# lunarlab-gatech/MorphSym-HGNN

Hardware: AMD Instinct MI355X
Metric: graph-windows/sec fwd+bwd, A1-C2 GRF regression (higher is better)
Workload: dtype bf16; 1 GPU; A1-C2 GRF regression (3-D), h=128, L=3, T=150, 8192 windows/GPU, fwd+MSE+bwd, all parameter gradients; global_batch=8192, parallelism=dp1, rccl_ranks=0

## Files before the change

### morphsym_hgnn_amd/csrc/mshgnn.hip

```cpp
#include "mshgnn_slab.hpp"
#include "mshgnn_enc.hpp"
#include "mshgnn_launch.hpp"
extern "C" const char* mshgnn_last_error(void) { return g_err.c_str(); }
extern "C" const char* mshgnn_version(void) { return "mshgnn 0.5 (gfx950)"; }
extern "C" int mshgnn_abi_version(void) { return MSHGNN_ABI_VERSION; }
extern "C" size_t mshgnn_struct_size(int which) {
    switch (which) {
        case 0: return sizeof(mshgnn_desc);
        case 1: return sizeof(mshgnn_info);
        case 2: return sizeof(mshgnn_ws_layout);
        case 3: return sizeof(mshgnn_window_desc);
        case 4: return sizeof(mshgnn_kernel_stat);
        case 5: return sizeof(mshgnn_mlp_desc);
        case 6: return sizeof(mshgnn_mlp_info);
        case 7: return sizeof(mshgnn_mlp_input);
        default: return 0;
    }
}


template <typename T> __device__ __forceinline__ void prep_one(const PrepArgs& a, int idx, bool with_bias) {
    constexpr int EPC = Prec<T>::EPC, NBV = Prec<T>::NBV;
    const int vec_per_pack = H * H / EPC;
    const int npk = a.pack_n < 0 ? a.n_packs : a.pack_n;
// ... 912 lines not shown

#ifndef GW_WPS
#define GW_WPS 3
#endif

template <bool ALIGNED, bool SERIES = false> __global__ __launch_bounds__(256, GW_WPS) void k_gradw_bf16_lean(GradwArgs a) {
    static_assert(!SERIES || ALIGNED, "the series gather replaces the aligned raw loads");
    using T = __bf16;
    __shared__ __attribute__((aligned(16))) __bf16 Ps[GWB_KW * GWB_PITCH];
    __shared__ __attribute__((aligned(16))) __bf16 Qs[GWB_KW * GWB_PITCH];
    __shared__ __attribute__((aligned(16))) u32x4 mlut[256];
    __shared__ __attribute__((aligned(16))) u32x4 qkeep_t[16];
    __shared__ __attribute__((aligned(16))) u32x4 qsign_t[GW_IPL][16];
    __shared__ unsigned long long sbase[GW_IPL][4];
    __shared__ unsigned long long sser[SERIES ? GW_IPL : 1][16][2];
    const int tid = threadIdx.x, lane = tid & 63, wv = __builtin_amdgcn_readfirstlane(tid >> 6);
    mlut[tid] = chunk_mask_bits<__bf16>(u32x4{0xffffffffu, 0xffffffffu, 0xffffffffu, 0xffffffffu}, (unsigned)tid);
    const int wr = wv >> 1, wc = wv & 1;
    const int ln = a.lane_order[blockIdx.x % a.n_pad], part = blockIdx.x / a.n_pad;
    if (ln < 0) return;
    const int* lh = a.lanes + ln * LANE_INTS;
    const int it0 = lh[0], nit = lh[1] - lh[0], bias_flag = lh[3];
    const int* im0 = a.items + it0 * ITEM_INTS;
    const int nchunks = (a.B + GWB_KW - 1) / GWB_KW;
    const int ch0 = (int)((int64_t)part * nchunks / a.n_parts), ch1 = (int)((int64_t)(part + 1) * nchunks / a.n_parts);
    const int nsteps = ch1 - ch0, total = nsteps * nit;
    const int c = tid & 15, r4 = (tid >> 4) * 4;

    const bool p_masked = im0[9] >= 0, q_raw = im0[4] < 0;
    const int ntile = (a.B + 15) >> 4;
    const unsigned voffP = (unsigned)(r4 * H + c * 8) * (unsigned)sizeof(T);
    const unsigned voffM = (unsigned)(((c >> 2) * ntile + (r4 >> 4)) * 64 + (c & 3) * 16 + (r4 & 15));
    const int qt = q_raw ? im0[3] - BUF_IN : 0;
    const unsigned qsb = q_raw ? (unsigned)(a.nodes[qt] * a.pitch[qt]) * (unsigned)sizeof(T) : (unsigned)(H * sizeof(T));
// ... 163 lines not shown
        for (int e = 0; e < 8; ++e) red[(r4 >> 2) * H + c * 8 + e] = bsum[e];
        __syncthreads();
        if (tid < H) {
            float s2 = 0.f;
#pragma unroll
            for (int r = 0; r < 16; ++r) s2 += red[r * H + tid];
            slab[H * H + tid] = s2;
        }
    }
}


#ifndef FIN_LB
#define FIN_LB 4
#endif
__global__ __launch_bounds__(256) void k_finalize(FinArgs a) {
    const int* f = a.fin + blockIdx.x * FIN_INTS;
    const int64_t dst = (int64_t)(unsigned)f[0] | ((int64_t)f[1] << 32);
    const int rows = f[2], cols = f[3], ld = f[4], tg = f[5], kind = f[6];
    const int* more = f[7] ? a.fin0 + f[7] : nullptr;
    const int RPB = (rows + gridDim.y - 1) / gridDim.y;
    const int r0 = blockIdx.y * RPB, r1 = min(rows, r0 + RPB);
    const int n = (r1 - r0) * cols;
    if (a.loss && blockIdx.x == 0 && blockIdx.y == 0 && threadIdx.x < 64) {
        float l = 0.f;
        for (int b = threadIdx.x; b < a.n_dec; b += 64) l += a.dec_slabs[(size_t)b * DEC_SLAB_FLOATS + 8 * H + 8];
#pragma unroll
        for (int m = 32; m >= 1; m >>= 1) l += __shfl_xor(l, m, 64);
        if (threadIdx.x == 0) *a.loss = l * a.inv_n + (a.accumulate ? *a.loss : 0.f);
    }
    if (!a.grad) return;
// ... 260 lines not shown
    if (prep_use_tiled(a.n_packs)) hipLaunchKernelGGL((k_prep_tiled<T, false>), dim3(prep_tiled_grid(a.n_packs, a.n_biases)), dim3(256), 0, st, a);
    else hipLaunchKernelGGL(k_prep<T>, dim3(prep_grid(a, Prec<T>::EPC, biases)), dim3(256), 0, st, a);
}
int launch_prep(const PrepArgs& a, bool split, hipStream_t st) {
    if (split) x3_launch_prep(a, true, st); else launch_prep_t<__bf16>(a, true, st);
    return MSHGNN_OK;
}

int run_finalize(const mshgnn_plan* p, const StepCall& c, const mshgnn_ws_layout& lay, int gw_parts) {
    const HostPlan& hp = p->hp;
    const mshgnn_desc& d = hp.d;
    char* ws = c.ws; float* gparams = c.grad_params; hipStream_t st = c.stream;
    const int B = (int)c.batch, gw_phase = c.gw_phase;
    float* loss = c.loss != LossKind::NONE ? c.loss_out : nullptr;
    FinArgs a{p->d_tables + hp.fin_off, p->d_tables + hp.fin_off, p->d_tables + hp.tgt_off, reinterpret_cast<const float*>(ws + lay.slabs),
              reinterpret_cast<const float*>(ws + lay.dec_slabs), gparams, hp.n_lanes, gw_parts, loss,
              1.0f / (float)(c.total_windows() * d.type_nodes[d.out_type] * (c.loss == LossKind::CE ? 1 : d.out_channels)),
              c.dec_done ? (int)((B + TILE_ROWS - 1) / TILE_ROWS) : NWG_DEC, c.accumulates()};
    int f0 = 0, nf = hp.n_fin;
    if (gw_phase == 0) nf = hp.n_fin_ph0;
    if (gw_phase == 1) { f0 = hp.n_fin_ph0; nf = hp.n_fin - hp.n_fin_ph0; a.loss = nullptr; }
    a.fin += (size_t)f0 * FIN_INTS;
    if (!gparams) {
        if (loss) hipLaunchKernelGGL(k_finalize, dim3(1, 1), dim3(256), 0, st, a);
        HIPCHK(hipGetLastError());
        return MSHGNN_OK;
    }
    ProfScope ps(p, hp.ks_fin, st);
    if (nf > 0) hipLaunchKernelGGL(k_finalize, dim3(nf, 64), dim3(256), 0, st, a);
    HIPCHK(hipGetLastError());
    return MSHGNN_OK;
}

template <typename T> static constexpr LaunchTraits plan_traits{
    (int)sizeof(T), Prec<T>::EPC, Prec<T>::EPC, Prec<T>::BLK, Prec<T>::ENC_MB * Prec<T>::ROWS, Prec<T>::ENC_MB * Prec<T>::BLK, sizeof(T) == 4 ? GW_KW : GWB_KW,
     false,  sizeof(T) == 2,  sizeof(T) == 2,  false,  sizeof(T) == 2,
    "the fused window assembly needs 16-byte aligned window rows (pitch a multiple of 8)",
    "wide source rows: the plan-dtype rows need 16-byte alignment and a pitch that is a multiple of 8"};

template <typename T>
static int forward_impl(const mshgnn_plan* p, StepCall& c) {
    const HostPlan& hp = p->hp;
    const mshgnn_desc& d = hp.d;
    const LaunchTraits& tr = plan_traits<T>;
// ... 77 lines not shown
    for (int l = hp.L - 1; l >= 0 && !fused_done; --l) {
        LayerArgs a{};
        a.x_in = ws + lay.dx[l + 1]; a.x_out = ws + lay.dx[l]; a.maskbits = reinterpret_cast<unsigned*>(ws + lay.mask[l]);
        a.hb = ws + lay.hb[l]; a.t1 = ws + lay.t1[l]; a.dh = ws + lay.dh[l]; a.du = ws + lay.du[l]; a.x_act = ws + lay.x[0];
        a.wpack = ws + lay.wpack; a.bias = reinterpret_cast<const float*>(ws + lay.bias);
        a.prog = p->d_tables + hp.bwd_prog_off[l]; a.B = B; a.NN = hp.NN; a.n_mlp = std::max(1, hp.n_mlp);
        a.dbg = p->dbg;
        ProfScope ps(p, hp.ks_layer_bwd0 + (hp.L - 1 - l), st);
        hipLaunchKernelGGL(k_layer_bwd<T>, dim3(tiles), dim3(LAYER_THREADS), hp.n_blk * Prec<T>::BLK, st, a);
    }
    const int gw_parts = gw_parts_for(hp.n_parts, hp.n_lanes, hp.gw_ipl, B, tr.gw_windows, p->n_cu);
    if (c.grad_params) {
        GradwArgs a{};
        fill_gradw_args(p, c, lay, tr, gw_parts, a);
        ProfScope ps(p, hp.ks_gradw, st);
        const dim3 grid(std::max(a.n_pad, 0) * gw_parts);
        if (a.n_pad <= 0) {}
        else if constexpr (sizeof(T) == 4) hipLaunchKernelGGL(k_gradw_f32, grid, dim3(256), 0, st, a);
        else if (c.gradw_from_series && c.series) hipLaunchKernelGGL((k_gradw_bf16_lean<true, true>), grid, dim3(256), 0, st, a);
        else if (a.aligned) hipLaunchKernelGGL(k_gradw_bf16_lean<true>, grid, dim3(256), 0, st, a);
        else hipLaunchKernelGGL(k_gradw_bf16_lean<false>, grid, dim3(256), 0, st, a);
    }
    return run_finalize(p, c, lay, gw_parts);
}

static int run_forward(const mshgnn_plan* p, StepCall& c) {
    if (c.wide && c.series) return set_err(MSHGNN_EINVAL, "a call takes its encoder rows from wide sources or from a series, not from both");
    if (p->gen) return gen_forward(p, c);
    if (p->hp.d.dtype == MSHGNN_BF16X3) return x3_forward(p, c);
    if (p->hp.d.dtype == MSHGNN_F32) return forward_impl<float>(p, c);
    return forward_impl<__bf16>(p, c);
}
// ... 452 lines not shown
```

### morphsym_hgnn_amd/csrc/mshgnn_device.hpp

```cpp
#pragma once
#include <type_traits>
#include <hip/hip_runtime.h>

#include <cmath>
#include <cstdio>
#include <cstdlib>
#include <cstring>
#include <string>
#include <vector>

#include "mshgnn_plan.hpp"

using namespace mshgnn;

typedef float f32x4 __attribute__((ext_vector_type(4)));
typedef float f32x2 __attribute__((ext_vector_type(2)));
typedef float f32x16 __attribute__((ext_vector_type(16)));
typedef __bf16 bf16x8 __attribute__((ext_vector_type(8)));
typedef unsigned int u32x4 __attribute__((ext_vector_type(4)));
typedef double f64x2 __attribute__((ext_vector_type(2)));
typedef unsigned int u32x2 __attribute__((ext_vector_type(2)));

#ifndef ENC_NT
#define ENC_NT 0
// ... 1229 lines not shown
template <typename T, int THREADS, bool SPLIT = false, bool TOLDS = false>
__device__ __forceinline__ void decoder_tail(const StackArgs& a, char* smem, int tid, int lane, int wv, int w0, int B) {
    if (a.dout <= 4) decoder_tail_impl<T, THREADS, 4, SPLIT, TOLDS>(a, smem, tid, lane, wv, w0, B);
    else decoder_tail_impl<T, THREADS, 8, SPLIT, TOLDS>(a, smem, tid, lane, wv, w0, B);
}
constexpr int DEC_NPP_STATIC = 4;

struct DecArgs {
    const void* xl; void* dxl; const float* params; const float* out_mask; float* out; const float* gout; float* slabs;
    int64_t off_w, off_b; int B, NN, node0, n_out, dout, slab0;
    const float* y; float* loss; float inv_n;
    const int32_t* labels;
};


struct GradwArgs {
    const char* ws; size_t buf_off[BUF_COUNT];
    const void* x[MSHGNN_MAX_TYPES]; int64_t pitch[MSHGNN_MAX_TYPES]; int nodes[MSHGNN_MAX_TYPES]; int vb[MSHGNN_MAX_TYPES];
    const int* items; const int* lanes; const int* lane_order; const uint8_t* signs; float* slabs; int B, n_lanes, n_parts, n_pad;
    int aligned;
    int dbg; long long* stamps;
    SeriesSrc ser;
};

constexpr int GWB_KW = 64;
constexpr int GWB_PITCH = 128;
__device__ __forceinline__ int gwb_elem(int row, int col) { return row * GWB_PITCH + ((((col >> 3) ^ ((row & 3) << 2)) << 3) | (col & 7)); }
typedef short s16x4 __attribute__((ext_vector_type(4)));

__device__ __forceinline__ bf16x8 tr_frag(const __bf16* tile, int w_base, int col_base, int lane) {
    const int g = lane >> 4, q = (lane >> 2) & 3, pp = lane & 3;
    const __bf16* p0 = tile + gwb_elem(w_base + 8 * (g >> 1) + q, col_base + 16 * (g & 1) + 4 * pp);
    const s16x4 lo = __builtin_amdgcn_ds_read_tr16_b64_v4i16((__attribute__((address_space(3))) s16x4*)(p0));
    const s16x4 hi = __builtin_amdgcn_ds_read_tr16_b64_v4i16((__attribute__((address_space(3))) s16x4*)(p0 + 4 * GWB_PITCH));
    typedef short s16x8 __attribute__((ext_vector_type(8)));
    const s16x8 v = {lo[0], lo[1], lo[2], lo[3], hi[0], hi[1], hi[2], hi[3]};
    return __builtin_bit_cast(bf16x8, v);
}


struct FinArgs { const int* fin; const int* fin0; const int* targets; const float* slabs; const float* dec_slabs; float* grad; int n_lanes, n_parts; float* loss; float inv_n;
                 int n_dec; int accumulate; };

struct mshgnn_gen_state;
struct ProfRec { int slot; hipEvent_t a, b; };
struct mshgnn_plan {
    HostPlan hp;
    bool prof = false;
    std::vector<ProfRec> recs;
    std::vector<hipEvent_t> free_events;
    int* d_tables = nullptr; uint8_t* d_signs = nullptr; float* d_out_mask = nullptr;
    PackDesc* d_packs = nullptr; BiasDesc* d_biases = nullptr;
    int* d_ig_nodes = nullptr;
    bool attr_set = false;
    bool use_fused = false;
    bool use_slab = false;
    bool slab_force = false; int n_cu = 256;
// ... 116 lines not shown
```

### morphsym_hgnn_amd/csrc/mshgnn_hostplan.cpp

```cpp
#include "mshgnn_plan.hpp"
#include "mshgnn_gen_plan.hpp"
#include "mshgnn_pick.hpp"

using namespace mshgnn;

namespace {
thread_local std::string g_hp_err;

std::string check_tables(const HostPlan& p) {
    char buf[256];
    auto bad = [&](const char* what, int l, int v, int lim) { snprintf(buf, sizeof buf, "%s: layer %d value %d limit %d", what, l, v, lim); return std::string(buf); };
    const int n_packs = (int)p.packs.size() * (p.split ? 2 : 1), n_bias = (int)p.biases.size();
    auto check_prog = [&](int off, int hs, int cb, int nblk, const char* what, int l) -> std::string {
        const int32_t* pr = p.tables.data() + off;
        if (off < 0 || off + FPROG_LEN > (int)p.tables.size()) return bad("program offset", l, off, (int)p.tables.size());
        auto at = [&](int i) { return (pr[128 + (i >> 2)] >> ((i & 3) << 3)) & 0xff; };
        const int nseg = at(0);
        if (nseg > 64) return bad("segments", l, nseg, 64);
        int pb = 1;
        for (int s = 0; s < nseg; ++s) {
            if (pr[s] < 0 || pr[s] >= n_packs) return bad(what, l, pr[s], n_packs);
            for (int u = 0; u < hs; ++u) pb += (pr[64 + s] >> (cb * u)) & ((1 << cb) - 1);
            if (hs * cb < 32 && (pr[64 + s] >> (hs * cb)) != 0) return bad("count bits beyond the slots", l, pr[64 + s], 0);
        }
// ... 105 lines not shown
    for (int i = 0; i < n_items; ++i) {
        const int32_t* it = T + p.item_off + i * GITEM_INTS;
        if (it[I_PBUF] < 0 || it[I_PBUF] >= GBUF_COUNT) return bad("item P buffer", i, it[I_PBUF], GBUF_COUNT);
        if (it[I_SRC0] < 0 || it[I_NSRC] < 1 || it[I_SRC0] + it[I_NSRC] > n_srcs) return bad("item source range", i, it[I_SRC0] + it[I_NSRC], n_srcs);
        { const std::string e = check_srcs(it[I_SRC0], it[I_NSRC], it[I_KIND], "item", i); if (!e.empty()) return e; }
    }
    return "";
}
}

extern "C" {

const char* mshgnn_hostplan_last_error() { return g_hp_err.c_str(); }

enum { HPM_OK = 0, HPM_L, HPM_NN, HPM_NMLP, HPM_FUSED, HPM_SLAB, HPM_SL_HB, HPM_SL_BLK, HPM_FS_BLK, HPM_NTABLES, HPM_NPACKS, HPM_NBIASES, HPM_SL_ALIAS, HPM_NITEMS, HPM_NLANES, HPM_NFIN,
       HPM_SL_FWD = 16, HPM_SL_BWD = 32, HPM_FS_FWD = 48, HPM_FS_BWD = 64, HPM_LIVE = 80 , HPM_NEED = 112, HPM_X3_ALIAS = 144, HPM_SPLIT = 145, HPM_COUNT = 160 };

int mshgnn_hostplan_compile(const mshgnn_desc* desc, int32_t* tables, int cap, int32_t* meta, int check) {
    HostPlan hp;
    if (!compile_plan(desc, hp)) { g_hp_err = hp.err; return -1; }
    if (check) { const std::string e = check_tables(hp); if (!e.empty()) { g_hp_err = "table check: " + e; return -2; } }
    if (meta) {
        std::memset(meta, 0, sizeof(int32_t) * HPM_COUNT);
        meta[HPM_OK] = 1; meta[HPM_L] = hp.L; meta[HPM_NN] = hp.NN; meta[HPM_NMLP] = hp.n_mlp; meta[HPM_FUSED] = hp.fused; meta[HPM_SLAB] = hp.slab; meta[HPM_SL_HB] = hp.sl_hb;
        meta[HPM_SL_BLK] = hp.sl_blk; meta[HPM_FS_BLK] = hp.fs_blk; meta[HPM_NTABLES] = (int)hp.tables.size(); meta[HPM_NPACKS] = (int)hp.packs.size(); meta[HPM_NBIASES] = (int)hp.biases.size();
        meta[HPM_X3_ALIAS] = hp.x3_alias; meta[HPM_SPLIT] = hp.split;
        meta[HPM_SL_ALIAS] = hp.sl_alias; meta[HPM_NITEMS] = hp.n_items; meta[HPM_NLANES] = hp.n_lanes; meta[HPM_NFIN] = hp.n_fin;
        for (int l = 0; l < hp.L; ++l) {
            meta[HPM_SL_FWD + l] = hp.sl_fwd_off[l]; meta[HPM_SL_BWD + l] = hp.sl_bwd_off[l]; meta[HPM_FS_FWD + l] = hp.fs_fwd_off[l]; meta[HPM_FS_BWD + l] = hp.fs_bwd_off[l];
            uint64_t lv = 0, nd = 0;
            for (int n = 0; n < hp.NN; ++n) { lv |= (uint64_t)(hp.live_n[l][n] ? 1 : 0) << n; nd |= (uint64_t)(hp.need_n[l][n] ? 1 : 0) << n; }
            meta[HPM_LIVE + 2 * l] = (int32_t)(uint32_t)lv; meta[HPM_LIVE + 2 * l + 1] = (int32_t)(uint32_t)(lv >> 32);
            meta[HPM_NEED + 2 * l] = (int32_t)(uint32_t)nd; meta[HPM_NEED + 2 * l + 1] = (int32_t)(uint32_t)(nd >> 32);
        }
    }
    if (tables) std::memcpy(tables, hp.tables.data(), sizeof(int32_t) * std::min<size_t>(cap > 0 ? cap : 0, hp.tables.size()));
    return (int)hp.tables.size();
}

int mshgnn_hostplan_compile_gen(const mshgnn_desc* desc, int32_t* meta, int check) {
    gen::GenPlan gp;
    if (!gen::compile_gen_plan(desc, gp)) { g_hp_err = gp.err; return -1; }
// ... 66 lines not shown
```

### morphsym_hgnn_amd/csrc/mshgnn_launch.hpp

```cpp
#pragma once
#include "mshgnn_device.hpp"
#include "mshgnn_pick.hpp"

struct LaunchTraits {
    int in_bytes;
    int in_epc;
    int pack_epc;
    int blk;
    int enc_windows;
    int enc_lds;
    int gw_windows;
    bool split;
    bool embed_prep;
    bool src_routes;
    bool wide_needs_rows;
    bool gradw_series;
    const char* series_rows_err;
    const char* wide_rows_err;
};

inline int plan_packs(const HostPlan& hp, const LaunchTraits& tr) { return tr.split ? hp.n_img : (int)hp.packs.size(); }

using PrepLaunch = void (*)(const PrepArgs&, bool biases, hipStream_t);
inline unsigned prep_grid(const PrepArgs& a, int pack_epc, bool biases) {
// ... 120 lines not shown
inline int forward_op(const StepCall& c) { return c.dec_done ? pick::OP_FWD_LOSS : c.training ? pick::OP_FWD_TRAIN : pick::OP_FWD_EVAL; }
inline void apply_stack_pick(const HostPlan& hp, const pick::StackPick& pk, const mshgnn_ws_layout& lay, StackArgs& a) {
    const int* fwd = pk.slab_prog ? hp.sl_fwd_off : hp.fs_fwd_off;
    const int* bwd = pk.slab_prog ? hp.sl_bwd_off : hp.fs_bwd_off;
    for (int l = 0; l < hp.L; ++l) { a.prog_off[l] = pk.what == pick::BWD ? bwd[l] : fwd[l]; if (pk.what == pick::STEP) a.prog_off_b[l] = bwd[l]; }
    if (pk.what != pick::FWD) a.mask0_off = lay.dd[0];
    a.red_off = pk.red_off; a.stash_nt = pk.stash_nt; a.stagger = pk.stagger;
}
inline int launch_stack(StackKernelFn kernel, const pick::StackPick& pk, hipStream_t st, const StackArgs& a) {
    if (!kernel) return set_err(MSHGNN_EHIP, std::string("no kernel in the launch table for ") + pick::kernel_name(pk.family, pk.k));
    hipLaunchKernelGGL(kernel, dim3(pk.tiles), dim3(pk.threads), pk.lds, st, a);
    HIPCHK(hipGetLastError());
    return MSHGNN_OK;
}

inline void fill_gradw_args(const mshgnn_plan* p, const StepCall& c, const mshgnn_ws_layout& lay, const LaunchTraits& tr, int gw_parts, GradwArgs& a) {
    const HostPlan& hp = p->hp;
    const mshgnn_desc& d = hp.d;
    a.ws = c.ws;
    for (int l = 0; l <= hp.L; ++l) { a.buf_off[BUF_X + l] = lay.x[l]; a.buf_off[BUF_DX + l] = lay.dx[l]; }
    for (int l = 0; l < hp.L; ++l) a.buf_off[BUF_MASK + l] = lay.mask[l];
    for (int l = 0; l < hp.L; ++l) { a.buf_off[BUF_DH + l] = lay.dh[l]; a.buf_off[BUF_HB + l] = lay.hb[l]; a.buf_off[BUF_T1 + l] = lay.t1[l]; a.buf_off[BUF_DU + l] = lay.du[l]; }
    for (int t = 0; t < hp.NT; ++t) {
        a.x[t] = c.x ? c.x[t] : nullptr; a.pitch[t] = c.x_pitch ? c.x_pitch[t] : d.type_width[t]; a.nodes[t] = d.type_nodes[t];
        a.vb[t] = vec_bytes(a.x[t], a.pitch[t], tr.in_bytes);
        if (t == 0) a.aligned = 1;
        if (a.vb[t] != 16 || a.pitch[t] % tr.in_epc) a.aligned = 0;
    }
    if (tr.gradw_series && c.gradw_from_series && c.series) a.ser = *c.series;
    a.items = p->d_tables + hp.item_off; a.lanes = p->d_tables + hp.lane_off; a.lane_order = p->d_tables + hp.lane_order_off; a.n_pad = hp.n_lanes_pad;
    if (c.gw_phase >= 0) { a.lane_order = p->d_tables + hp.order_ph_off[c.gw_phase]; a.n_pad = hp.npad_ph[c.gw_phase]; }
    a.signs = p->d_signs; a.slabs = reinterpret_cast<float*>(c.ws + lay.slabs); a.B = (int)c.batch; a.n_lanes = hp.n_lanes; a.n_parts = gw_parts;
}
```

### morphsym_hgnn_amd/csrc/mshgnn_plan.hpp

```cpp
#pragma once
#include <algorithm>
#include <array>
#include <cmath>
#include <cstdint>
#include <cstdio>
#include <cstring>
#include <string>
#include <vector>

#include "../../include/mshgnn.h"

#ifdef MSHGNN_TUNING
#define TUNE_ENV(name) std::getenv(name)
#else
#define TUNE_ENV(name) (static_cast<const char*>(nullptr))
#endif

namespace mshgnn {

constexpr int H = 128;
constexpr int GMAX = 12;
constexpr int TILE_ROWS = 16;
constexpr int MAX_L = 16;
#ifndef LDS_LIMIT_KB
// ... 36 lines not shown
       FH_SLOTA = 8 + 4 * FS_MAXN,
       FH_SLOTB = FH_SLOTA + 16,
       FH_SIZE = FH_SLOTB + 16,
       FH_NEXT = FH_SLOTA };
static_assert(FH_NEXT + 8 + 20 <= FH_SIZE && MSHGNN_MAX_TYPES <= 4, "header: next-layer array");
constexpr int SL_HA = 12, SL_HB = 6, SL_HB_MAX = 8, SL_THREADS = 256;
constexpr int SL_CBA = 2, SL_CBB = 3;
enum { FF_RESIDUAL = 1, FF_ENC_MASK = 2, FF_SCR_ALIAS = 4, FF_A_EMPTY = 8, FF_B_EMPTY = 16 };

enum { BUF_X = 0, BUF_DX = 17, BUF_DH = 34, BUF_HB = 50, BUF_T1 = 66, BUF_DU = 82, BUF_IN = 98, BUF_MASK = 102, BUF_COUNT = 118 };
constexpr int ITEM_INTS = 10;
constexpr int TGT_INTS = 8;
constexpr int LANE_INTS = 4;
constexpr int FIN_INTS = 8;
enum { FIN_MATRIX = 0, FIN_BIAS = 1, FIN_ZERO = 2, FIN_DEC_W = 3, FIN_DEC_B = 4 };

struct PackDesc {
    int orient;
    int n_src;
    int64_t src[8];
    int ld;
    int col0;
    int ncols;
};
struct BiasDesc { int n_src; int64_t src[8]; };

struct HostPlan {
    mshgnn_desc d{};
    void* jit_prog = nullptr;
    std::vector<int32_t> rel_src, rel_dst, rel_mean, rel_edge_off, edges;
// ... 30 lines not shown
    std::vector<int32_t> tables;
    int fwd_prog_off[MAX_L]{}, bwd_prog_off[MAX_L]{};
    bool fused = false;
    int fs_fwd_off[MAX_L]{}, fs_bwd_off[MAX_L]{};
    bool slab = false;
    int sl_fwd_off[MAX_L]{}, sl_bwd_off[MAX_L]{}, sl_ta = -1, sl_hb = SL_HB, sl_blk = 0;
    bool sl_alias = false;
    int fs_blk = 0;
    bool x3_alias = false;
    int ks_stack_fwd = -1, ks_stack_bwd = -1;
    int item_off = 0, n_items = 0, tgt_off = 0, n_targets = 0, lane_off = 0, n_lanes = 0, n_parts = 1, n_wg_gradw = 0;
    int lane_order_off = 0, n_lanes_pad = 0, gw_ipl = 1;
    int order_ph_off[2]{}, npad_ph[2]{}, n_fin_ph0 = 0;
    int64_t grad_split = -1;
    int fin_off = 0, n_fin = 0;
    int enc_tile_mb = 4;
    int n_slabs = 0;
    std::vector<float> out_mask_f;
    std::vector<mshgnn_kernel_stat> kstats;
    int ks_prep = 0, ks_enc = 0, ks_layer_fwd0 = 0, ks_dec_fwd = 0, ks_dec_bwd = 0, ks_layer_bwd0 = 0, ks_gradw = 0, ks_fin = 0, ks_stack_step = 0;
    mshgnn_info info{};
    std::string err;
};

inline bool fail(HostPlan& p, const std::string& m) { p.err = m; return false; }

inline int add_pack(HostPlan& p, int orient, const std::vector<int64_t>& src, int ld, int col0, int ncols) {
    PackDesc q{}; q.orient = orient; q.n_src = (int)src.size(); q.ld = ld; q.col0 = col0; q.ncols = ncols;
    for (size_t i = 0; i < src.size(); ++i) q.src[i] = src[i];
    p.packs.push_back(q); return (int)p.packs.size() - 1;
// ... 843 lines not shown
        std::vector<int32_t> extra;
        for (auto& f : fins) {
            if (!is_ph1(f)) ++p.n_fin_ph0;
            if (is_ph1(f) && f.target >= 0 && !tgt_is_enc[f.target]) p.grad_split = -1;
            for (int64_t m : f.more) if ((p.grad_split >= 0 && m < p.grad_split) != is_ph1(f)) p.grad_split = -1;
            T.push_back((int32_t)(f.dst & 0xffffffff)); T.push_back((int32_t)(f.dst >> 32)); T.push_back(f.rows); T.push_back(f.cols);
            T.push_back(f.ld); T.push_back(f.target); T.push_back(f.kind);
            T.push_back(f.more.empty() ? 0 : (int32_t)(fins.size() * FIN_INTS + extra.size()));
            if (!f.more.empty()) {
                extra.push_back((int32_t)f.more.size());
                for (int64_t m : f.more) { extra.push_back((int32_t)(m & 0xffffffff)); extra.push_back((int32_t)(m >> 32)); }
            }
        }
        T.insert(T.end(), extra.begin(), extra.end());
        if (p.grad_split < 0) p.n_fin_ph0 = p.n_fin;
    }

    p.info.rows_per_tile = p.rows; p.info.total_nodes = p.NN; p.info.lds_bytes = (int64_t)p.n_blk * p.blk_bytes;
    p.info.flops_fwd = alg_fwd; p.info.flops_bwd = alg_bwd; p.info.flops_exec_fwd = exec_fwd; p.info.flops_exec_bwd = exec_bwd;
    double bytes = 0, bytes_all = 0;
    for (int t = 0; t < NT; ++t) { bytes += (double)enc_n[t] * d.type_width[t] * (p.split ? 4 : p.esize); bytes_all += (double)d.type_nodes[t] * d.type_width[t] * (p.split ? 4 : p.esize); }
    p.info.bytes_in = bytes_all; p.info.bytes_in_live = bytes; p.info.n_gradw_workgroups = p.n_wg_gradw;
    p.info.n_launches_fwd = 3 + L; p.info.n_launches_bwd = 3 + L;
    p.info.grad_split = p.grad_split;
    p.info.kernel_sets = (p.fused ? 1 : 0) | (p.slab ? 2 : 0);

    {
        const double es = p.esize * p.planes, act = (double)p.enc_live_nodes * H * es;
        auto add = [&](const std::string& name, int bound, double fa, double fe, double by) {
            mshgnn_kernel_stat k{}; std::snprintf(k.name, sizeof(k.name), "%s", name.c_str());
// ... 59 lines not shown
```

### morphsym_hgnn_amd/csrc/mshgnn_x3.hip

```cpp
#include "mshgnn_x3_stack.hpp"
#include "mshgnn_enc.hpp"
#include "mshgnn_launch.hpp"

__device__ __forceinline__ void prep_one_x3(const PrepArgs& a, int idx, bool with_bias) {
    constexpr int EPC = 8, NBV = 8;
    const int vec_per_pack = H * H / EPC;
    const int npk = a.pack_n < 0 ? a.n_packs : a.pack_n;
    const int total = npk * vec_per_pack;
    if (idx < total) {
        const int pack = a.pack0 + idx / vec_per_pack, r = idx % vec_per_pack;
        const int gid = pack * vec_per_pack + r;
        const int lane = r % 64, v = (r / 64) % NBV, wv = r / (64 * NBV);
        const PackDesc pd = a.packs[pack];
        float g[8][EPC];
#pragma unroll
        for (int i = 0; i < 8; ++i)
#pragma unroll
            for (int x = 0; x < EPC; ++x) {
                const int i16 = lane & 15;
                const int k = 32 * (lane >> 4) + 8 * (v & 3) + x, col = wv * 32 + 8 * (i16 >> 2) + 4 * (v >> 2) + (i16 & 3);
                g[i][x] = 0.f;
                if (i < pd.n_src) {
                    if (pd.orient == 0) { if (k < pd.ncols) g[i][x] = a.params[pd.src[i] + (int64_t)col * pd.ld + pd.col0 + k]; }
                    else g[i][x] = a.params[pd.src[i] + (int64_t)k * pd.ld + col];
// ... 124 lines not shown
#ifndef GWX3_WPS
#define GWX3_WPS 3
#endif

template <bool ALIGNED> __global__ __launch_bounds__(256, GWX3_WPS) void k_gradw_x3_lean(GradwArgs a) {
    using T = T16;
    constexpr int KW = 32;
    __shared__ __attribute__((aligned(16))) __bf16 Ph[KW * GWB_PITCH];
    __shared__ __attribute__((aligned(16))) __bf16 Pl[KW * GWB_PITCH];
    __shared__ __attribute__((aligned(16))) __bf16 Qh[KW * GWB_PITCH];
    __shared__ __attribute__((aligned(16))) __bf16 Ql[KW * GWB_PITCH];
    __shared__ __attribute__((aligned(16))) u32x4 mlut[256];
    __shared__ __attribute__((aligned(16))) u32x4 qfix[16][2];
    __shared__ __attribute__((aligned(16))) u32x4 qsign_t[GW_IPL][16][2];
    __shared__ unsigned long long sbase[GW_IPL][4];
    const int tid = threadIdx.x, lane = tid & 63, wv = __builtin_amdgcn_readfirstlane(tid >> 6);
    mlut[tid] = chunk_mask_bits<__bf16>(u32x4{0xffffffffu, 0xffffffffu, 0xffffffffu, 0xffffffffu}, (unsigned)tid);
    const int wr = wv >> 1, wc = wv & 1;
    const int ln = a.lane_order[blockIdx.x % a.n_pad], part = blockIdx.x / a.n_pad;
    if (ln < 0) return;
    const int* lh = a.lanes + ln * LANE_INTS;
    const int it0 = lh[0], nit = lh[1] - lh[0], bias_flag = lh[3];
    const int* im0 = a.items + it0 * ITEM_INTS;
    const int nchunks = (a.B + KW - 1) / KW;
    const int ch0 = (int)((int64_t)part * nchunks / a.n_parts), ch1 = (int)((int64_t)(part + 1) * nchunks / a.n_parts);
    const int nsteps = ch1 - ch0, total = nsteps * nit;
    const int c = tid & 15, r2 = (tid >> 4) * 2;
    constexpr int ROWB = 2 * H * (int)sizeof(T);

    const bool p_masked = im0[9] >= 0, q_act = im0[4] >= 0;
    const int ntile = (a.B + 15) >> 4;
    const unsigned voffP = (unsigned)(r2 * ROWB + c * 16);
    const unsigned voffM = (unsigned)(((c >> 2) * ntile + (r2 >> 4)) * 64 + (c & 3) * 16 + (r2 & 15));
    const int qt = q_act ? 0 : im0[3] - BUF_IN;
// ... 262 lines not shown
    }
    if (c.gw_phase != 1 && !c.stack_done) {
        StackArgs a{};
        x3_stack_args(p, c, lay, a);
        a.tile_in = c.ws + lay.dx[hp.L]; a.training = 1;
        const pick::StackPick pk = pick::pick_stack(stack_query(p, c, pick::PLAN_X3, pick::OP_BWD, tr.blk, a));
        apply_stack_pick(hp, pk, lay, a);
        ProfScope ps(p, hp.ks_stack_bwd, st);
        if (int rc = launch_stack(x3_stack_kernel(hp, pk), pk, st, a)) return rc;
    }
    const int gw_parts = gw_parts_for(hp.n_parts, hp.n_lanes, hp.gw_ipl, B, tr.gw_windows, p->n_cu);
    if (c.grad_params) {
        GradwArgs a{};
        fill_gradw_args(p, c, lay, tr, gw_parts, a);
        ProfScope ps(p, hp.ks_gradw, st);
        if (a.n_pad <= 0) {}
        else if (a.aligned) hipLaunchKernelGGL(k_gradw_x3_lean<true>, dim3(a.n_pad * gw_parts), dim3(256), 0, st, a);
        else hipLaunchKernelGGL(k_gradw_x3_lean<false>, dim3(a.n_pad * gw_parts), dim3(256), 0, st, a);
    }
    return run_finalize(p, c, lay, gw_parts);
}
```

Baseline: 44.83 million windows/s.

## Move decoder-gradient, zeroing and loss work into extra gradw workgroups; slim finalize

Adds side workgroups to the weight-gradient kernels that zero unused gradient regions, reduce decoder weight/bias gradients and compute the loss, so that work overlaps with the main gradw blocks. For non-f32 plans, finalize becomes a lighter per-row-slab kernel that only reduces the MATRIX/BIAS slabs across lanes and parts, using float4 loads. The old finalize is kept as k_finalize_whole for f32 and loss-only paths. The cost targeted is finalize's serial tail and its large 2-D grid, paid for with extra plan tables and a branch at the start of every gradw block.

```diff
diff --git a/morphsym_hgnn_amd/csrc/mshgnn.hip b/morphsym_hgnn_amd/csrc/mshgnn.hip
--- a/morphsym_hgnn_amd/csrc/mshgnn.hip
+++ b/morphsym_hgnn_amd/csrc/mshgnn.hip
@@ -950,10 +950,13 @@
     __shared__ __attribute__((aligned(16))) u32x4 qsign_t[GW_IPL][16];
     __shared__ unsigned long long sbase[GW_IPL][4];
     __shared__ unsigned long long sser[SERIES ? GW_IPL : 1][16][2];
+    const int sw = (int)blockIdx.x - a.side.wg0;
+    if (sw >= 0 && sw < a.side.n_grid) { if (sw < a.side.n) gw_side_workgroup(a.side, sw); return; }
+    const int bx = (int)blockIdx.x - a.side.main0;
     const int tid = threadIdx.x, lane = tid & 63, wv = __builtin_amdgcn_readfirstlane(tid >> 6);
     mlut[tid] = chunk_mask_bits<__bf16>(u32x4{0xffffffffu, 0xffffffffu, 0xffffffffu, 0xffffffffu}, (unsigned)tid);
     const int wr = wv >> 1, wc = wv & 1;
-    const int ln = a.lane_order[blockIdx.x % a.n_pad], part = blockIdx.x / a.n_pad;
+    const int ln = a.lane_order[bx % a.n_pad], part = bx / a.n_pad;
     if (ln < 0) return;
     const int* lh = a.lanes + ln * LANE_INTS;
     const int it0 = lh[0], nit = lh[1] - lh[0], bias_flag = lh[3];
@@ -1147,7 +1150,57 @@
 #ifndef FIN_LB
 #define FIN_LB 4
 #endif
-__global__ __launch_bounds__(256) void k_finalize(FinArgs a) {
+__global__ __launch_bounds__(256) void k_finalize(FinSlabArgs a) {
+    const int* f = a.recs + (size_t)blockIdx.x * FSLAB_INTS;
+    const int64_t dst = (int64_t)(unsigned)f[0] | ((int64_t)f[1] << 32);
+    const int row0 = f[2], rows = f[3], cols = f[4], ld = f[5], l0 = f[6], nl = f[7], kind = f[9];
+    const int* more = f[8] ? a.fin0 + f[8] : nullptr;
+    const int rr = threadIdx.x >> 5, c0 = (threadIdx.x & 31) * 4;
+    if (rr >= rows || c0 >= cols) return;
+    const int r = row0 + rr;
+    const float* sp = a.slabs + (size_t)l0 * SLAB_FLOATS + (kind == FIN_MATRIX ? r * H : H * H) + c0;
+    const size_t pstride = (size_t)a.n_lanes * SLAB_FLOATS;
+    float4 s = float4{0.f, 0.f, 0.f, 0.f};
+    for (int j0 = 0; j0 < nl; j0 += FIN_LB)
+        for (int p0 = 0; p0 < a.n_parts; p0 += 4) {
+            float4 v[FIN_LB][4];
+#pragma unroll
+            for (int jj = 0; jj < FIN_LB; ++jj)
+#pragma unroll
+                for (int pp = 0; pp < 4; ++pp)
+                    v[jj][pp] = (j0 + jj < nl && p0 + pp < a.n_parts) ? *reinterpret_cast<const float4*>(sp + (size_t)(j0 + jj) * SLAB_FLOATS + (size_t)(p0 + pp) * pstride)
+                                                                       : float4{0.f, 0.f, 0.f, 0.f};
+#pragma unroll
+            for (int jj = 0; jj < FIN_LB; ++jj) {
+                s.x += (v[jj][0].x + v[jj][1].x) + (v[jj][2].x + v[jj][3].x);
+                s.y += (v[jj][0].y + v[jj][1].y) + (v[jj][2].y + v[jj][3].y);
+                s.z += (v[jj][0].z + v[jj][1].z) + (v[jj][2].z + v[jj][3].z);
+                s.w += (v[jj][0].w + v[jj][1].w) + (v[jj][2].w + v[jj][3].w);
+            }
+        }
+    const int64_t at = (int64_t)r * ld + c0;
+    float* g = a.grad + dst + at;
+    const bool full = c0 + 4 <= cols;
+    float e[4] = {s.x, s.y, s.z, s.w};
+    if (a.accumulate) {
+#pragma unroll
+        for (int k = 0; k < 4; ++k) if (c0 + k < cols) e[k] += g[k];
+    }
+    auto put = [&](float* q) {
+        if (full && ((uintptr_t)q & 15) == 0) *reinterpret_cast<float4*>(q) = float4{e[0], e[1], e[2], e[3]};
+        else {
+#pragma unroll
+            for (int k = 0; k < 4; ++k) if (c0 + k < cols) q[k] = e[k];
+        }
+    };
+    put(g);
+    if (more) {
+        const int nm = more[0];
+        for (int m = 0; m < nm; ++m) put(a.grad + (((int64_t)(unsigned)more[1 + 2 * m] | ((int64_t)more[2 + 2 * m] << 32)) + at));
+    }
+}
+
+__global__ __launch_bounds__(256) void k_finalize_whole(FinArgs a) {
     const int* f = a.fin + blockIdx.x * FIN_INTS;
     const int64_t dst = (int64_t)(unsigned)f[0] | ((int64_t)f[1] << 32);
     const int rows = f[2], cols = f[3], ld = f[4], tg = f[5], kind = f[6];
@@ -1438,20 +1491,27 @@
     const int B = (int)c.batch, gw_phase = c.gw_phase;
     float* loss = c.loss != LossKind::NONE ? c.loss_out : nullptr;
     FinArgs a{p->d_tables + hp.fin_off, p->d_tables + hp.fin_off, p->d_tables + hp.tgt_off, reinterpret_cast<const float*>(ws + lay.slabs),
-              reinterpret_cast<const float*>(ws + lay.dec_slabs), gparams, hp.n_lanes, gw_parts, loss,
-              1.0f / (float)(c.total_windows() * d.type_nodes[d.out_type] * (c.loss == LossKind::CE ? 1 : d.out_channels)),
-              c.dec_done ? (int)((B + TILE_ROWS - 1) / TILE_ROWS) : NWG_DEC, c.accumulates()};
+              reinterpret_cast<const float*>(ws + lay.dec_slabs), gparams, hp.n_lanes, gw_parts, loss, fin_inv_n(hp, c), fin_n_dec(c), c.accumulates()};
+    if (!gparams) {
+        if (loss) hipLaunchKernelGGL(k_finalize_whole, dim3(1, 1), dim3(256), 0, st, a);
+        HIPCHK(hipGetLastError());
+        return MSHGNN_OK;
+    }
+    ProfScope ps(p, hp.ks_fin, st);
+    if (fin_split(hp)) {
+        FinSlabArgs s{p->d_tables + hp.fslab_off, p->d_tables + hp.fin_off, a.slabs, gparams, hp.n_lanes, gw_parts, c.accumulates()};
+        int n = hp.n_fslab;
+        if (gw_phase == 0) n = hp.n_fslab_ph0;
+        if (gw_phase == 1) { s.recs += (size_t)hp.n_fslab_ph0 * FSLAB_INTS; n = hp.n_fslab - hp.n_fslab_ph0; }
+        if (n > 0) hipLaunchKernelGGL(k_finalize, dim3(n), dim3(256), 0, st, s);
+        HIPCHK(hipGetLastError());
+        return MSHGNN_OK;
+    }
     int f0 = 0, nf = hp.n_fin;
     if (gw_phase == 0) nf = hp.n_fin_ph0;
     if (gw_phase == 1) { f0 = hp.n_fin_ph0; nf = hp.n_fin - hp.n_fin_ph0; a.loss = nullptr; }
     a.fin += (size_t)f0 * FIN_INTS;
-    if (!gparams) {
-        if (loss) hipLaunchKernelGGL(k_finalize, dim3(1, 1), dim3(256), 0, st, a);
-        HIPCHK(hipGetLastError());
-        return MSHGNN_OK;
-    }
-    ProfScope ps(p, hp.ks_fin, st);
-    if (nf > 0) hipLaunchKernelGGL(k_finalize, dim3(nf, 64), dim3(256), 0, st, a);
+    if (nf > 0) hipLaunchKernelGGL(k_finalize_whole, dim3(nf, 64), dim3(256), 0, st, a);
     HIPCHK(hipGetLastError());
     return MSHGNN_OK;
 }
@@ -1559,8 +1619,9 @@
         GradwArgs a{};
         fill_gradw_args(p, c, lay, tr, gw_parts, a);
         ProfScope ps(p, hp.ks_gradw, st);
-        const dim3 grid(std::max(a.n_pad, 0) * gw_parts);
-        if (a.n_pad <= 0) {}
+        const dim3 grid(a.side.n_grid + std::max(a.n_pad, 0) * gw_parts);
+        a.n_pad = std::max(a.n_pad, 1);
+        if (grid.x == 0) {}
         else if constexpr (sizeof(T) == 4) hipLaunchKernelGGL(k_gradw_f32, grid, dim3(256), 0, st, a);
         else if (c.gradw_from_series && c.series) hipLaunchKernelGGL((k_gradw_bf16_lean<true, true>), grid, dim3(256), 0, st, a);
         else if (a.aligned) hipLaunchKernelGGL(k_gradw_bf16_lean<true>, grid, dim3(256), 0, st, a);
diff --git a/morphsym_hgnn_amd/csrc/mshgnn_device.hpp b/morphsym_hgnn_amd/csrc/mshgnn_device.hpp
--- a/morphsym_hgnn_amd/csrc/mshgnn_device.hpp
+++ b/morphsym_hgnn_amd/csrc/mshgnn_device.hpp
@@ -1267,7 +1267,10 @@
 };
 
 
+struct GwSide { const int* recs; int n, n_grid, wg0, main0; const float* dec_slabs; float* grad; float* loss; float inv_n; int n_dec; int accumulate; };
+
 struct GradwArgs {
+    GwSide side;
     const char* ws; size_t buf_off[BUF_COUNT];
     const void* x[MSHGNN_MAX_TYPES]; int64_t pitch[MSHGNN_MAX_TYPES]; int nodes[MSHGNN_MAX_TYPES]; int vb[MSHGNN_MAX_TYPES];
     const int* items; const int* lanes; const int* lane_order; const uint8_t* signs; float* slabs; int B, n_lanes, n_parts, n_pad;
@@ -1294,6 +1297,47 @@
 
 struct FinArgs { const int* fin; const int* fin0; const int* targets; const float* slabs; const float* dec_slabs; float* grad; int n_lanes, n_parts; float* loss; float inv_n;
                  int n_dec; int accumulate; };
+struct FinSlabArgs { const int* recs; const int* fin0; const float* slabs; float* grad; int n_lanes, n_parts, accumulate; };
+
+__device__ __forceinline__ void gw_side_workgroup(const GwSide& s, int wg) {
+    const int tid = threadIdx.x, lane = tid & 63;
+    if (s.loss && wg == 0 && tid < 64) {
+        float l = 0.f;
+        for (int b = tid; b < s.n_dec; b += 64) l += s.dec_slabs[(size_t)b * DEC_SLAB_FLOATS + 8 * H + 8];
+#pragma unroll
+        for (int m = 32; m >= 1; m >>= 1) l += __shfl_xor(l, m, 64);
+        if (tid == 0) *s.loss = l * s.inv_n + (s.accumulate ? *s.loss : 0.f);
+    }
+    const int* f = s.recs + (size_t)wg * SIDE_INTS;
+    const int64_t dst = (int64_t)(unsigned)f[0] | ((int64_t)f[1] << 32);
+    const int cols = f[3], ld = f[4], kind = f[5];
+    if (kind == FIN_ZERO) {
+        const int rows = f[2];
+        const bool v4 = (((uintptr_t)s.grad | (uintptr_t)dst | (uintptr_t)ld) & 3) == 0 && ((uintptr_t)s.grad & 15) == 0;
+        const int nv = v4 ? cols >> 2 : 0;
+        for (int r = 0; r < rows; ++r) {
+            float* g = s.grad + dst + (int64_t)r * ld;
+            for (int i = tid; i < nv; i += 256) reinterpret_cast<float4*>(g)[i] = float4{0.f, 0.f, 0.f, 0.f};
+            for (int i = 4 * nv + tid; i < cols; i += 256) g[i] = 0.f;
+        }
+        return;
+    }
+    const bool is_mat = kind == FIN_DEC_W;
+    for (int e = f[2] + (tid >> 6); e < f[6]; e += 4) {
+        const int r = e / cols, cidx = e % cols;
+        const int src = is_mat ? r * H + cidx : 8 * H + cidx;
+        float sum = 0.f;
+        for (int b0 = 0; b0 < s.n_dec; b0 += 512) {
+            float v[8];
+#pragma unroll
+            for (int u = 0; u < 8; ++u) { const int b = b0 + lane + 64 * u; v[u] = b < s.n_dec ? s.dec_slabs[(size_t)b * DEC_SLAB_FLOATS + src] : 0.f; }
+            sum += ((v[0] + v[1]) + (v[2] + v[3])) + ((v[4] + v[5]) + (v[6] + v[7]));
+        }
+#pragma unroll
+        for (int m = 32; m >= 1; m >>= 1) sum += __shfl_xor(sum, m, 64);
+        if (lane == 0) { float* gp = s.grad + dst + (int64_t)r * ld + cidx; *gp = s.accumulate ? *gp + sum : sum; }
+    }
+}
 
 struct mshgnn_gen_state;
 struct ProfRec { int slot; hipEvent_t a, b; };
diff --git a/morphsym_hgnn_amd/csrc/mshgnn_hostplan.cpp b/morphsym_hgnn_amd/csrc/mshgnn_hostplan.cpp
--- a/morphsym_hgnn_amd/csrc/mshgnn_hostplan.cpp
+++ b/morphsym_hgnn_amd/csrc/mshgnn_hostplan.cpp
@@ -143,7 +143,8 @@
 const char* mshgnn_hostplan_last_error() { return g_hp_err.c_str(); }
 
 enum { HPM_OK = 0, HPM_L, HPM_NN, HPM_NMLP, HPM_FUSED, HPM_SLAB, HPM_SL_HB, HPM_SL_BLK, HPM_FS_BLK, HPM_NTABLES, HPM_NPACKS, HPM_NBIASES, HPM_SL_ALIAS, HPM_NITEMS, HPM_NLANES, HPM_NFIN,
-       HPM_SL_FWD = 16, HPM_SL_BWD = 32, HPM_FS_FWD = 48, HPM_FS_BWD = 64, HPM_LIVE = 80 , HPM_NEED = 112, HPM_X3_ALIAS = 144, HPM_SPLIT = 145, HPM_COUNT = 160 };
+       HPM_SL_FWD = 16, HPM_SL_BWD = 32, HPM_FS_FWD = 48, HPM_FS_BWD = 64, HPM_LIVE = 80 , HPM_NEED = 112, HPM_X3_ALIAS = 144, HPM_SPLIT = 145,
+       HPM_FIN_OFF = 146, HPM_NFIN_PH0, HPM_SIDE_OFF, HPM_NSIDE_DEC, HPM_NSIDE_Z0, HPM_NSIDE_Z1, HPM_FSLAB_OFF, HPM_NFSLAB, HPM_NFSLAB_PH0, HPM_TGT_OFF, HPM_SPLIT_LO, HPM_SPLIT_HI, HPM_COUNT = 160 };
 
 int mshgnn_hostplan_compile(const mshgnn_desc* desc, int32_t* tables, int cap, int32_t* meta, int check) {
     HostPlan hp;
@@ -155,6 +156,10 @@
         meta[HPM_SL_BLK] = hp.sl_blk; meta[HPM_FS_BLK] = hp.fs_blk; meta[HPM_NTABLES] = (int)hp.tables.size(); meta[HPM_NPACKS] = (int)hp.packs.size(); meta[HPM_NBIASES] = (int)hp.biases.size();
         meta[HPM_X3_ALIAS] = hp.x3_alias; meta[HPM_SPLIT] = hp.split;
         meta[HPM_SL_ALIAS] = hp.sl_alias; meta[HPM_NITEMS] = hp.n_items; meta[HPM_NLANES] = hp.n_lanes; meta[HPM_NFIN] = hp.n_fin;
+        meta[HPM_FIN_OFF] = hp.fin_off; meta[HPM_NFIN_PH0] = hp.n_fin_ph0; meta[HPM_SIDE_OFF] = hp.side_off; meta[HPM_NSIDE_DEC] = hp.n_side_dec;
+        meta[HPM_NSIDE_Z0] = hp.n_side_zero[0]; meta[HPM_NSIDE_Z1] = hp.n_side_zero[1]; meta[HPM_FSLAB_OFF] = hp.fslab_off; meta[HPM_NFSLAB] = hp.n_fslab;
+        meta[HPM_NFSLAB_PH0] = hp.n_fslab_ph0; meta[HPM_TGT_OFF] = hp.tgt_off;
+        meta[HPM_SPLIT_LO] = (int32_t)(uint32_t)(hp.grad_split & 0xffffffff); meta[HPM_SPLIT_HI] = (int32_t)(hp.grad_split >> 32);
         for (int l = 0; l < hp.L; ++l) {
             meta[HPM_SL_FWD + l] = hp.sl_fwd_off[l]; meta[HPM_SL_BWD + l] = hp.sl_bwd_off[l]; meta[HPM_FS_FWD + l] = hp.fs_fwd_off[l]; meta[HPM_FS_BWD + l] = hp.fs_bwd_off[l];
             uint64_t lv = 0, nd = 0;
diff --git a/morphsym_hgnn_amd/csrc/mshgnn_launch.hpp b/morphsym_hgnn_amd/csrc/mshgnn_launch.hpp
--- a/morphsym_hgnn_amd/csrc/mshgnn_launch.hpp
+++ b/morphsym_hgnn_amd/csrc/mshgnn_launch.hpp
@@ -158,6 +158,28 @@
     return MSHGNN_OK;
 }
 
+inline float fin_inv_n(const HostPlan& hp, const StepCall& c) {
+    const mshgnn_desc& d = hp.d;
+    return 1.0f / (float)(c.total_windows() * d.type_nodes[d.out_type] * (c.loss == LossKind::CE ? 1 : d.out_channels));
+}
+inline int fin_n_dec(const StepCall& c) { return c.dec_done ? (int)((c.batch + TILE_ROWS - 1) / TILE_ROWS) : NWG_DEC; }
+inline bool fin_split(const HostPlan& hp) { return hp.d.dtype != MSHGNN_F32; }
+
+inline void fill_gradw_side(const mshgnn_plan* p, const StepCall& c, const mshgnn_ws_layout& lay, int n_main, GwSide& s) {
+    const HostPlan& hp = p->hp;
+    s = GwSide{};
+    if (!fin_split(hp) || !c.grad_params) return;
+    int first = 0, n = hp.n_side_dec;
+    if (!c.accumulates()) n += hp.n_side_zero[0] + (c.gw_phase == 0 ? 0 : hp.n_side_zero[1]);
+    if (c.gw_phase == 1) { first = hp.n_side_dec + hp.n_side_zero[0]; n = c.accumulates() ? 0 : hp.n_side_zero[1]; }
+    static const int where = [] { const char* e = TUNE_ENV("MSHGNN_GW_SIDE"); return e ? atoi(e) : 0; }();
+    s.recs = p->d_tables + hp.side_off + (size_t)first * SIDE_INTS; s.n = n;
+    s.n_grid = where == 0 ? (n + 7) / 8 * 8 : n; s.wg0 = where == 1 ? n_main : 0; s.main0 = where == 1 ? 0 : s.n_grid;
+    s.dec_slabs = reinterpret_cast<const float*>(c.ws + lay.dec_slabs); s.grad = c.grad_params;
+    s.loss = c.loss != LossKind::NONE && c.gw_phase != 1 ? c.loss_out : nullptr;
+    s.inv_n = fin_inv_n(hp, c); s.n_dec = fin_n_dec(c); s.accumulate = c.accumulates();
+}
+
 inline void fill_gradw_args(const mshgnn_plan* p, const StepCall& c, const mshgnn_ws_layout& lay, const LaunchTraits& tr, int gw_parts, GradwArgs& a) {
     const HostPlan& hp = p->hp;
     const mshgnn_desc& d = hp.d;
@@ -175,4 +197,5 @@
     a.items = p->d_tables + hp.item_off; a.lanes = p->d_tables + hp.lane_off; a.lane_order = p->d_tables + hp.lane_order_off; a.n_pad = hp.n_lanes_pad;
     if (c.gw_phase >= 0) { a.lane_order = p->d_tables + hp.order_ph_off[c.gw_phase]; a.n_pad = hp.npad_ph[c.gw_phase]; }
     a.signs = p->d_signs; a.slabs = reinterpret_cast<float*>(c.ws + lay.slabs); a.B = (int)c.batch; a.n_lanes = hp.n_lanes; a.n_parts = gw_parts;
-}
+    fill_gradw_side(p, c, lay, std::max(a.n_pad, 0) * gw_parts, a.side);
+}
diff --git a/morphsym_hgnn_amd/csrc/mshgnn_plan.hpp b/morphsym_hgnn_amd/csrc/mshgnn_plan.hpp
--- a/morphsym_hgnn_amd/csrc/mshgnn_plan.hpp
+++ b/morphsym_hgnn_amd/csrc/mshgnn_plan.hpp
@@ -74,6 +74,12 @@
 constexpr int LANE_INTS = 4;
 constexpr int FIN_INTS = 8;
 enum { FIN_MATRIX = 0, FIN_BIAS = 1, FIN_ZERO = 2, FIN_DEC_W = 3, FIN_DEC_B = 4 };
+constexpr int SIDE_INTS = 8;
+constexpr int FSLAB_INTS = 10;
+constexpr int FSLAB_ROWS = 8;
+constexpr int SIDE_DEC_ELEMS = 8;
+constexpr int SIDE_ZERO_ELEMS = 8192;
+constexpr int SIDE_ZERO_ROWS = 64;
 
 struct PackDesc {
     int orient;
@@ -134,6 +140,8 @@
     int order_ph_off[2]{}, npad_ph[2]{}, n_fin_ph0 = 0;
     int64_t grad_split = -1;
     int fin_off = 0, n_fin = 0;
+    int side_off = 0, n_side_dec = 0, n_side_zero[2]{};
+    int fslab_off = 0, n_fslab = 0, n_fslab_ph0 = 0;
     int enc_tile_mb = 4;
     int n_slabs = 0;
     std::vector<float> out_mask_f;
@@ -1007,6 +1015,37 @@
         }
         T.insert(T.end(), extra.begin(), extra.end());
         if (p.grad_split < 0) p.n_fin_ph0 = p.n_fin;
+        auto lo32 = [](int64_t v) { return (int32_t)(v & 0xffffffff); };
+        auto hi32 = [](int64_t v) { return (int32_t)(v >> 32); };
+        p.side_off = (int)T.size(); p.n_side_dec = 0; p.n_side_zero[0] = p.n_side_zero[1] = 0;
+        auto side = [&](int64_t dst, int a, int cols, int ld, int kind, int last) { T.insert(T.end(), {lo32(dst), hi32(dst), a, cols, ld, kind, last, 0}); };
+        for (auto& f : fins)
+            if (f.kind == FIN_DEC_W || f.kind == FIN_DEC_B)
+                for (int e0 = 0; e0 < f.rows * f.cols; e0 += SIDE_DEC_ELEMS) { side(f.dst, e0, f.cols, f.ld, f.kind, std::min(f.rows * f.cols, e0 + SIDE_DEC_ELEMS)); ++p.n_side_dec; }
+        for (int ph = 0; ph < 2; ++ph)
+            for (size_t i = 0; i < fins.size(); ++i) {
+                const FinRec& f = fins[i];
+                if (f.kind != FIN_ZERO || ((int)i >= p.n_fin_ph0) != (ph == 1)) continue;
+                if (f.rows == 1 || f.cols == f.ld) {
+                    const int64_t n = (int64_t)f.rows * f.cols;
+                    for (int64_t o = 0; o < n; o += SIDE_ZERO_ELEMS) { const int m = (int)std::min<int64_t>(SIDE_ZERO_ELEMS, n - o); side(f.dst + o, 1, m, m, FIN_ZERO, 0); ++p.n_side_zero[ph]; }
+                } else {
+                    for (int r0 = 0; r0 < f.rows; r0 += SIDE_ZERO_ROWS) { side(f.dst + (int64_t)r0 * f.ld, std::min(SIDE_ZERO_ROWS, f.rows - r0), f.cols, f.ld, FIN_ZERO, 0); ++p.n_side_zero[ph]; }
+                }
+            }
+        p.fslab_off = (int)T.size(); p.n_fslab = p.n_fslab_ph0 = 0;
+        size_t xoff = fins.size() * FIN_INTS;
+        for (size_t i = 0; i < fins.size(); ++i) {
+            const FinRec& f = fins[i];
+            const int more = f.more.empty() ? 0 : (int32_t)xoff;
+            if (!f.more.empty()) xoff += 1 + 2 * f.more.size();
+            if (f.kind != FIN_MATRIX && f.kind != FIN_BIAS) continue;
+            for (int r0 = 0; r0 < f.rows; r0 += FSLAB_ROWS) {
+                T.insert(T.end(), {lo32(f.dst), hi32(f.dst), r0, std::min(FSLAB_ROWS, f.rows - r0), f.cols, f.ld, tgt_lane_begin[f.target], tgt_lane_end[f.target] - tgt_lane_begin[f.target], more, f.kind});
+                ++p.n_fslab;
+                if ((int)i < p.n_fin_ph0) ++p.n_fslab_ph0;
+            }
+        }
     }
 
     p.info.rows_per_tile = p.rows; p.info.total_nodes = p.NN; p.info.lds_bytes = (int64_t)p.n_blk * p.blk_bytes;
diff --git a/morphsym_hgnn_amd/csrc/mshgnn_x3.hip b/morphsym_hgnn_amd/csrc/mshgnn_x3.hip
--- a/morphsym_hgnn_amd/csrc/mshgnn_x3.hip
+++ b/morphsym_hgnn_amd/csrc/mshgnn_x3.hip
@@ -162,10 +162,13 @@
     __shared__ __attribute__((aligned(16))) u32x4 qfix[16][2];
     __shared__ __attribute__((aligned(16))) u32x4 qsign_t[GW_IPL][16][2];
     __shared__ unsigned long long sbase[GW_IPL][4];
+    const int sw = (int)blockIdx.x - a.side.wg0;
+    if (sw >= 0 && sw < a.side.n_grid) { if (sw < a.side.n) gw_side_workgroup(a.side, sw); return; }
+    const int bx = (int)blockIdx.x - a.side.main0;
     const int tid = threadIdx.x, lane = tid & 63, wv = __builtin_amdgcn_readfirstlane(tid >> 6);
     mlut[tid] = chunk_mask_bits<__bf16>(u32x4{0xffffffffu, 0xffffffffu, 0xffffffffu, 0xffffffffu}, (unsigned)tid);
     const int wr = wv >> 1, wc = wv & 1;
-    const int ln = a.lane_order[blockIdx.x % a.n_pad], part = blockIdx.x / a.n_pad;
+    const int ln = a.lane_order[bx % a.n_pad], part = bx / a.n_pad;
     if (ln < 0) return;
     const int* lh = a.lanes + ln * LANE_INTS;
     const int it0 = lh[0], nit = lh[1] - lh[0], bias_flag = lh[3];
@@ -458,9 +461,11 @@
         GradwArgs a{};
         fill_gradw_args(p, c, lay, tr, gw_parts, a);
         ProfScope ps(p, hp.ks_gradw, st);
-        if (a.n_pad <= 0) {}
-        else if (a.aligned) hipLaunchKernelGGL(k_gradw_x3_lean<true>, dim3(a.n_pad * gw_parts), dim3(256), 0, st, a);
-        else hipLaunchKernelGGL(k_gradw_x3_lean<false>, dim3(a.n_pad * gw_parts), dim3(256), 0, st, a);
+        const dim3 grid(a.side.n_grid + std::max(a.n_pad, 0) * gw_parts);
+        a.n_pad = std::max(a.n_pad, 1);
+        if (grid.x == 0) {}
+        else if (a.aligned) hipLaunchKernelGGL(k_gradw_x3_lean<true>, grid, dim3(256), 0, st, a);
+        else hipLaunchKernelGGL(k_gradw_x3_lean<false>, grid, dim3(256), 0, st, a);
     }
     return run_finalize(p, c, lay, gw_parts);
 }
```

Measured after the change: 46.25 million windows/s (median of 6 runs). +3.2%, better.
